# fwilliams/point-cloud-utils

Measured on AMD Instinct MI355X. Metric: query-points/s, Chamfer 1M-vs-1M fp32, higher is better.
Workload: dtype f32

## Files before the change

### point_cloud_utils_amd/csrc/grid2.h

```cpp
#pragma once
#include "grid.h"

namespace pcu {

constexpr int kPrepSamples = 1024;
constexpr int kXPartStride = 8;
constexpr int kStagedMaxBuckets = 2048;
constexpr int kFillWords = 2 * kStagedMaxBuckets + 8;

template <typename T>
struct CellMap {
    T org[3], inv_h; int G[3];
    __device__ __forceinline__ explicit CellMap(const GridParams<T>& g) {
#pragma unroll
        for (int j = 0; j < 3; ++j) { org[j] = uniform(g.org[j]); G[j] = uniform(g.G[j]); }
        inv_h = uniform(g.inv_h);
    }
    __device__ __forceinline__ unsigned cell(T x, T y, T z) const {
        const int cx = cell_coord(x, org[0], inv_h, G[0]), cy = cell_coord(y, org[1], inv_h, G[1]), cz = cell_coord(z, org[2], inv_h, G[2]);
        return (unsigned)row_run_lo(G[0], grid_row(G[1], cy, cz), cx, cx);
    }
};

__device__ __forceinline__ unsigned hash32(unsigned x) { x ^= x >> 16; x *= 0x7feb352du; x ^= x >> 15; x *= 0x846ca68bu; x ^= x >> 16; return x; }
// ... 285 lines not shown
        T rng6[6];
        const SampleOf<T> smp = sample_request<T>(a, a.n, tid);
        layout_from_sample<T>(a, a.n, smp, s_col, s_fin, &s_fresh, rng6);
        if (tid == 0) {
            GridGeo<T> f;
            for (int j = 0; j < 3; ++j) { f.org[j] = s_fresh.org[j]; f.slack[j] = s_fresh.slack[j]; f.G[j] = s_fresh.G[j]; f.rlo[j] = rng6[j]; f.rhi[j] = rng6[3 + j]; }
            f.h = s_fresh.h; f.inv_h = s_fresh.inv_h; f.ncells = s_fresh.ncells;
            if (a.geo_in) {
                const GridGeo<T> u = *a.geo_in;
                bool stale = false;
                for (int j = 0; j < 3; ++j) {
                    const T eu = u.rhi[j] - u.rlo[j], ef = f.rhi[j] - f.rlo[j], ext = eu > ef ? eu : ef, tol = (T)0.05 * ext;
                    const T dl = f.rlo[j] - u.rlo[j], dh = f.rhi[j] - u.rhi[j];
                    if (!((dl < (T)0 ? -dl : dl) <= tol) || !((dh < (T)0 ? -dh : dh) <= tol)) stale = true;
                }
                const T hr = f.h / u.h;
                if (!(hr > (T)0.96 && hr < (T)1.04)) stale = true;
                s_stale = stale ? 1 : 0;
            }
            *a.geo_out = f;
        }
        __syncthreads();
    }
    for (int i = tid; i < a.n_zero_next; i += kSortThreads) a.zero_next[i] = 0ull;
    for (int i = tid; i < a.n_zero2; i += kSortThreads) a.zero2[i] = 0u;
    T lo[3] = {Limits<T>::max_v, Limits<T>::max_v, Limits<T>::max_v};
    T hi[3] = {-Limits<T>::max_v, -Limits<T>::max_v, -Limits<T>::max_v};
    unsigned nf = 0;
    for (int b = tid; b < a.n_xpart; b += kSortThreads) {
#pragma unroll
        for (int j = 0; j < 3; ++j) {
            const T p = a.xpartial[(size_t)b * kXPartStride + j], q = a.xpartial[(size_t)b * kXPartStride + 3 + j];
            lo[j] = p < lo[j] ? p : lo[j]; hi[j] = q > hi[j] ? q : hi[j];
        }
        nf |= (unsigned)a.xpartial[(size_t)b * kXPartStride + 6];
    }
#pragma unroll
    for (int j = 0; j < 3; ++j) {
        const T p = wave_min63(lo[j]), q = wave_max63(hi[j]);
        if (lane == 63) { s_lo[wave][j] = p; s_hi[wave][j] = q; }
    }
    { const unsigned m = wave_or63(nf); if (lane == 63) s_nf[wave] = m; }
    __syncthreads();
    if (tid != 0) return;
    GridParams<T>* gp = a.gp;
    unsigned m = 0;
    for (int w = 0; w < kSortThreads / 64; ++w) m |= s_nf[w];
    const unsigned pinf = (m >> 1) & 7u, ninf = (m >> 4) & 7u;
    gp->nonfinite = ((m & 1u) ? kNfNaN : 0) | ((pinf & ninf) ? kNfBothInf : 0) | ((pinf | ninf) ? kNfAnyInf : 0) | (int)(m << 8);
    for (int j = 0; j < 3; ++j) {
        T p = s_lo[0][j], q = s_hi[0][j];
        for (int w = 1; w < kSortThreads / 64; ++w) { p = s_lo[w][j] < p ? s_lo[w][j] : p; q = s_hi[w][j] > q ? s_hi[w][j] : q; }
        if (!(p <= q)) { p = 0; q = 0; }
        gp->gmin[j] = p; gp->gmax[j] = q;
    }
    gp->has_large = (*a.ovf ? 2 : 0) | (s_stale ? kGeoStale : 0);
    if (a.n_large) *a.n_large = 0u;
    put_sentinels(a.sorted, a.n);
}

constexpr int kHeadTrips = (kStagedMaxBuckets + kSortThreads - 1) / kSortThreads;
template <typename T>
__device__ __forceinline__ void sort2_head_request(const Build2Side<T>& a, const int b, unsigned long long (&fw)[kHeadTrips]) {
#pragma unroll
    for (int q = 0; q < kHeadTrips; ++q) { const int i = q * kSortThreads + (int)threadIdx.x; fw[q] = i < b ? a.fill[i] : 0ull; }
}
__device__ __forceinline__ unsigned sort2_head_fold(const unsigned long long (&fw)[kHeadTrips], unsigned* const s_cnt, const int CB, unsigned* const s_w) {
    const int tid = threadIdx.x, lane = tid & 63, wave = tid >> 6;
    unsigned part = 0;
#pragma unroll
    for (int q = 0; q < kHeadTrips; ++q) part += (unsigned)(fw[q] >> 32);
#pragma unroll
    for (int o = 32; o > 0; o >>= 1) part += __shfl_xor(part, o, 64);
    if (lane == 0) s_w[wave] = part;
    for (int i = tid; i < CB; i += kSortThreads) s_cnt[i] = 0u;
    __syncthreads();
    unsigned s = 0;
    for (int w = 0; w < kSortThreads / 64; ++w) s += s_w[w];
    __syncthreads();
    return s;
}

constexpr int kRegIters = (kStageRecs + kSortThreads - 1) / kSortThreads;
template <typename T, bool FAST>
__device__ __forceinline__ void sort2_body(const int b, const Build2Side<T>& a, const int cnt_cap, const unsigned long long (&hw)[kHeadTrips], const unsigned pf, const unsigned nvalid,
                                           unsigned* const s_cnt, Pt4<T>* const s_stage, unsigned* const s_w, unsigned long long* const s_q, long long t_prev) {
    GridParams<T>* const gp = a.gp;
    const CellMap<T> cm(*gp);
    const int ncells = uniform(gp->ncells);
    const int shift = a.shift, CB = 1 << shift;
    const int NB = (ncells + CB - 1) >> shift;
    const int tid = threadIdx.x, lane = tid & 63, wave = tid >> 6;
    long long* const prof = a.prof;
#define S2_PROF(slot) do { if (prof && tid == 0) { const long long t_now = wall_clock64(); atomicAdd((unsigned long long*)&prof[slot], (unsigned long long)(t_now - t_prev)); t_prev = t_now; } } while (0)
    const unsigned cap = a.cap;
    const unsigned c0 = (unsigned)b << shift;
    const int ncl = min(CB, ncells - (int)c0);
    const Pt4<T>* const slot = a.tmp + (size_t)b * cap;
    const unsigned lastp = pf ? pf - 1u : 0u;
    typedef typename RawRec<T>::type Raw;
    constexpr int kIters = FAST ? kRegIters : kSortIters;
    constexpr int kSortBatch = 4;
    Raw recs[FAST ? kRegIters : 1];
    unsigned rr[kIters];
    if (FAST) {
        const Raw* const rslot = reinterpret_cast<const Raw*>(slot);
#pragma unroll
        for (int u = 0; u < kRegIters; ++u) recs[u] = rslot[min((unsigned)(u * kSortThreads + tid), lastp)];
    }
    const unsigned s = sort2_head_fold(hw, s_cnt, CB, s_w);
    const unsigned e = s + nvalid;
    S2_PROF(0);
    if (FAST) {
#pragma unroll
        for (int u = 0; u < kRegIters; ++u) {
            const unsigned p = (unsigned)(u * kSortThreads + tid);
            const Pt4<T>& rec = reinterpret_cast<const Pt4<T>&>(recs[u]);
            rr[u] = 0xffffffffu;
            if (p < pf && rec.idx >= 0) {
                const unsigned c = cm.cell(rec.x, rec.y, rec.z) - c0;
                rr[u] = (c << 16) | atomicAdd(&s_cnt[c], 1u);
            }
        }
    } else {
#pragma unroll
        for (int it0 = 0; it0 < kIters; it0 += kSortBatch) {
            Pt4<T> rec[kSortBatch];
            const bool batch_on = (unsigned)(it0 * kSortThreads) < pf;
            if (batch_on) {
#pragma unroll
                for (int u = 0; u < kSortBatch; ++u) rec[u] = slot[min((unsigned)((it0 + u) * kSortThreads + tid), lastp)];
            }
#pragma unroll
            for (int u = 0; u < kSortBatch; ++u) {
                const unsigned p = (unsigned)((it0 + u) * kSortThreads + tid);
                rr[it0 + u] = 0xffffffffu;
                if (batch_on && p < pf && rec[u].idx >= 0) {
                    const unsigned c = cm.cell(rec[u].x, rec[u].y, rec[u].z) - c0;
                    rr[it0 + u] = (c << 16) | atomicAdd(&s_cnt[c], 1u);
                }
            }
        }
    }
    __syncthreads();
    S2_PROF(1);
    const int per = CB >= kSortThreads ? CB / kSortThreads : 1;
    const int i0 = tid * per;
    {
        unsigned v[kBkMaxCellsPerBucket / kSortThreads], sum = 0; unsigned long long sq = 0;
#pragma unroll
        for (int q = 0; q < kBkMaxCellsPerBucket / kSortThreads; ++q) {
            v[q] = (q < per && i0 + q < CB) ? s_cnt[i0 + q] : 0u;
            sum += v[q]; sq += (unsigned long long)v[q] * v[q];
        }
        unsigned inc = sum;
#pragma unroll
        for (int o = 1; o < 64; o <<= 1) { const unsigned t = __shfl_up(inc, o, 64); if (lane >= o) inc += t; }
#pragma unroll
        for (int o = 32; o > 0; o >>= 1) sq += __shfl_xor(sq, o, 64);
        if (lane == 63) s_w[wave] = inc;
        if (lane == 0) s_q[wave] = sq;
        __syncthreads();
        if (tid == 0) {
            unsigned run = 0; unsigned long long Q = 0;
            for (int w = 0; w < kSortThreads / 64; ++w) { const unsigned t = s_w[w]; s_w[w] = run; run += t; Q += s_q[w]; }
            if (Q) atomicAdd(&gp->sumsq, Q);
            if (b == NB - 1) a.cell_start[ncells] = e;
        }
        __syncthreads();
        unsigned ex = inc - sum + s_w[wave];
#pragma unroll
        for (int q = 0; q < kBkMaxCellsPerBucket / kSortThreads; ++q) {
            if (q < per && i0 + q < CB) {
                s_cnt[i0 + q] = ex;
                if (i0 + q < ncl) a.cell_start[c0 + i0 + q] = s + ex;
                ex += v[q];
            }
        }
    }
    __syncthreads();
    S2_PROF(2);
    const int n_pts = a.n;
    T* const xyz = xyz_of(a.sorted, n_pts);
    int* const idx32 = idx32_of(a.sorted, n_pts);
    if (!FAST) {
#pragma unroll
        for (int it0 = 0; it0 < kIters; it0 += kSortBatch) {
            if (!((unsigned)(it0 * kSortThreads) < pf)) break;
            Pt4<T> rec[kSortBatch];
#pragma unroll
            for (int u = 0; u < kSortBatch; ++u) rec[u] = slot[min((unsigned)((it0 + u) * kSortThreads + tid), lastp)];
#pragma unroll
            for (int u = 0; u < kSortBatch; ++u) {
                const unsigned r = rr[it0 + u];
                if (r != 0xffffffffu) {
                    const unsigned pos = s + s_cnt[r >> 16] + (r & 0xffffu);
                    if (a.want_pt4) a.sorted[pos] = rec[u];
                    put_xyz(a.sorted, n_pts, pos, rec[u]);
                }
            }
        }
        return;
    }
    constexpr unsigned V = 16 / sizeof(T);
    T* const st = reinterpret_cast<T*>(s_stage);
    int* const sidx0 = reinterpret_cast<int*>(st + (V + 3 * kStageRecs + V - 1) / V * V);
    static_assert(((V + 3 * kStageRecs + V - 1) / V * V) * sizeof(T) + ((size_t)kStageRecs + 4) * 4 <= (size_t)kStageRecs * sizeof(Pt4<T>) + 64, "both streams fit the stage (bucket_sort_lds_bytes)");
    const unsigned phase = (unsigned)((3ull * (unsigned long long)s) & (V - 1));
    const unsigned iph = (unsigned)((reinterpret_cast<size_t>(idx32 + s) >> 2) & 3u);
    int* const sidx = sidx0 + iph;
    {
#pragma unroll
        for (int u = 0; u < kRegIters; ++u) {
            const unsigned r = rr[u];
            if (r != 0xffffffffu) {
                const Pt4<T>& rec = reinterpret_cast<const Pt4<T>&>(recs[u]);
                const unsigned pos = s_cnt[r >> 16] + (r & 0xffffu);
                T* const o = st + phase + 3u * pos;
                o[0] = rec.x; o[1] = rec.y; o[2] = rec.z; sidx[pos] = (int)rec.idx;
            }
        }
    }
    __syncthreads();
    S2_PROF(3);
    if (a.want_pt4) {
        for (unsigned i = tid; i < nvalid; i += kSortThreads) { Pt4<T> r; const T* const o = st + phase + 3u * i; r.x = o[0]; r.y = o[1]; r.z = o[2]; r.idx = sidx[i]; a.sorted[s + i] = r; }
    }
    {
        const unsigned end = phase + 3u * nvalid;
        T* const out = xyz + (3 * (size_t)s - phase);
        const unsigned v0 = (phase + V - 1) / V, v1 = end / V;
        for (unsigned c = v0 + tid; c < v1; c += kSortThreads)
            store16_wt(reinterpret_cast<Chunk16*>(out) + c, reinterpret_cast<const Chunk16*>(st)[c]);
        if (tid < V) {
            const unsigned La = phase + tid;
            if (La < min(v0 * V, end)) out[La] = st[La];
            const unsigned Lb = max(v1 * V, v0 * V) + tid;
            if (v1 >= v0 && Lb < end) out[Lb] = st[Lb];
        }
    }
    {
        const unsigned iend = iph + nvalid;
        int* const iout = idx32 + s - iph;
        const unsigned w0 = (iph + 3u) / 4u, w1 = iend / 4u;
        for (unsigned c = w0 + tid; c < w1; c += kSortThreads)
            store16_wt(reinterpret_cast<Chunk16*>(iout) + c, reinterpret_cast<const Chunk16*>(sidx0)[c]);
        if (tid >= 64 && tid < 68) {
            const unsigned t = (unsigned)tid - 64u;
            const unsigned La = iph + t;
            if (La < min(w0 * 4u, iend)) iout[La] = sidx0[La];
            const unsigned Lb = max(w1 * 4u, w0 * 4u) + t;
            if (w1 >= w0 && Lb < iend) iout[Lb] = sidx0[Lb];
        }
    }
    S2_PROF(4);
    if (prof) { asm volatile("s_waitcnt vmcnt(0)" ::: "memory"); S2_PROF(5); if (tid == 0) atomicAdd((unsigned long long*)&prof[7], 1ull); }
#undef S2_PROF
}

template <typename T>
__device__ __forceinline__ void sort2_bucket(const int b, const Build2Side<T>& a, const int cnt_cap) {
    extern __shared__ __attribute__((aligned(32))) unsigned char s_dyn[];
    unsigned* const s_cnt = reinterpret_cast<unsigned*>(s_dyn);
    Pt4<T>* const s_stage = reinterpret_cast<Pt4<T>*>(s_dyn + (size_t)cnt_cap * 4);
    __shared__ unsigned s_w[kSortThreads / 64 + 1];
    __shared__ unsigned long long s_q[kSortThreads / 64];
    if (*a.ovf) return;
    const int CB = 1 << a.shift;
    const int NB = (uniform(a.gp->ncells) + CB - 1) >> a.shift;
    if (b >= NB) return;
    long long t_prev = a.prof ? wall_clock64() : 0;
    const unsigned long long fw = a.fill[b];
    unsigned long long hw[kHeadTrips];
    sort2_head_request<T>(a, b, hw);
    const unsigned pf = min((unsigned)uniform(fw), a.cap), nvalid = (unsigned)(uniform(fw) >> 32);
    static_assert(kSortThreads * kSortIters >= kLargeBucket, "one trip per record of a full slot");
    if (pf <= (unsigned)(kRegIters * kSortThreads) && nvalid <= (unsigned)kStageRecs) sort2_body<T, true>(b, a, cnt_cap, hw, pf, nvalid, s_cnt, s_stage, s_w, s_q, t_prev);
    else sort2_body<T, false>(b, a, cnt_cap, hw, pf, nvalid, s_cnt, s_stage, s_w, s_q, t_prev);
}

template <typename T>
__global__ __launch_bounds__(kSortThreads) void k_bucket_sort2(const Build2Args<T> p, int nb0, int nb1, int cnt_cap, int nfold) {
    const int bid = (int)blockIdx.x;
    if (bid < nfold) { fold_xpartials<T>(p.a[bid]); return; }
    const int b = bid - nfold;
    const int side = b >= nb0 ? 1 : 0;
    sort2_bucket<T>(side ? b - nb0 : b, p.a[side], cnt_cap);
}

template <typename T>
struct Pt4Side { Pt4<T>* sorted; int n; };
template <typename T>
__global__ __launch_bounds__(kBlock) void k_make_pt4(const Pt4Side<T> a0, const Pt4Side<T> a1, int nb0) {
    const bool second = (int)blockIdx.x >= nb0;
    const Pt4Side<T>& a = second ? a1 : a0;
    const int nblk = second ? (int)gridDim.x - nb0 : nb0, bid = second ? (int)blockIdx.x - nb0 : (int)blockIdx.x;
    const T* const xyz = xyz_of(a.sorted, a.n);
    const int* const idx32 = idx32_of(a.sorted, a.n);
    for (int i = bid * kBlock + (int)threadIdx.x; i < a.n + 8; i += nblk * kBlock) {
        Pt4<T> r; r.x = xyz[3 * (size_t)i]; r.y = xyz[3 * (size_t)i + 1]; r.z = xyz[3 * (size_t)i + 2]; r.idx = idx32[i];
        a.sorted[i] = r;
    }
}

}
```

### point_cloud_utils_amd/csrc/index_host.h

```cpp
#pragma once

template <typename T>
struct GridIndex {
    GridParams<T>* gp = nullptr;
    unsigned* cell_start = nullptr;
    Pt4<T>* sorted = nullptr;
    unsigned* cell_of = nullptr; unsigned* rank = nullptr; unsigned* block_sums = nullptr;
    T* bbox_partial = nullptr;
    int n = 0, max_cells = 0, scan_blocks = 0;
    bool bucketed = false; int shift = 0, nb_max = 0, n_zero = 0;
    double h_want = 0.0;
    Pt4<T>* tmp = nullptr; unsigned *bucket_total = nullptr, *bucket_start = nullptr, *block_base = nullptr, *large_list = nullptr, *n_large = nullptr;
    bool one_pass = false;
    T* xpartial = nullptr;
    bool lean = false;
    const T* src = nullptr; double occ_built = 0.0;
    bool shared_grid = false;
};

static int max_cells_for(int64_t n, double occ) {
    double c = (double)n / (occ > 0 ? occ : 1.0) * 1.25 + 64.0;
    if (c > 64.0 * 1024 * 1024) c = 64.0 * 1024 * 1024;
    return (int)c;
}
// ... 25 lines not shown
    if (aalloc(a, &g.cell_start, (size_t)g.max_cells + 1 + kBkMaxBuckets + 8 + 64)) return -1;
    g.cell_start += 64;
    if (a.alloc((void**)&g.sorted, sorted_records_bytes((size_t)n, sizeof(Pt4<T>), sizeof(T)))) return -1;
    if (aalloc(a, &g.cell_of, (size_t)n)) return -1;
    if (aalloc(a, &g.rank, (size_t)n)) return -1;
    if (aalloc(a, &g.block_sums, (size_t)g.scan_blocks + 1)) return -1;
    if (aalloc(a, &g.bbox_partial, (size_t)kBboxBlocks * kBboxStride)) return -1;
    g.n_zero = g.max_cells + 1;
    if (g.bucketed) {
        g.bucket_total = g.cell_start + g.max_cells + 1; g.n_large = g.bucket_total + g.nb_max; g.n_zero = g.max_cells + 1 + g.nb_max + 1;
        g.one_pass = one_pass;
        if (aalloc(a, &g.tmp, one_pass ? std::max((size_t)n, (size_t)g.nb_max * kLargeBucket) : (size_t)n)) return -1;
        if (aalloc(a, &g.bucket_start, (size_t)g.nb_max + 1) || aalloc(a, &g.large_list, (size_t)g.nb_max + 1)) return -1;
        if (aalloc(a, &g.block_base, (size_t)((n + kBkBlockPts - 1) / kBkBlockPts) * g.nb_max)) return -1;
        if (one_pass && aalloc(a, &g.xpartial, (size_t)((n + 2047) / 2048) * kXPartStride)) return -1;
    }
    return 0;
}
template <typename T>
static size_t index_bytes(int64_t n, double occ) {
    ArenaState count; count.cap = ~(size_t)0 >> 1;
    Arena a(&count); GridIndex<T> g;
    (void)index_alloc(a, g, n, occ, IndexFor::OnePass);
    return count.off;
}
template <typename T>
static void index_same_form(GridIndex<T>& a, GridIndex<T>& b) {
    if (a.bucketed && b.bucketed && a.one_pass != b.one_pass) a.one_pass = b.one_pass = false;
}

template <typename T>
static GridSide<T> grid_side(const GridIndex<T>& g) {
    GridSide<T> r{};
    r.gp = g.gp; r.partial = g.bbox_partial; r.nparts = kBboxBlocks; r.n = g.n; r.occupancy = g.occ_built; r.max_cells = g.max_cells;
    r.sentinel = g.sorted + g.n; r.h_want = g.h_want; r.pts = g.src;
    return r;
}
template <typename T>
static BboxSide<T> bbox_side(const GridIndex<T>& g, void* zero2, int n_zero2) {
    BboxSide<T> r{};
    r.pts = g.src; r.n = g.n; r.partial = g.bbox_partial; r.counts = g.cell_start; r.n_counts = g.n_zero;
    r.zero2 = (unsigned*)zero2; r.n_zero2 = n_zero2; r.gp = g.gp;
    return r;
}
template <typename T>
static BucketSide<T> bucket_side(const GridIndex<T>& g) {
    BucketSide<T> r{};
    r.pts = g.src; r.n = g.n; r.gp = g.gp; r.shift = g.shift; r.nb_stride = g.nb_max;
    r.bucket_total = g.bucket_total; r.block_base = g.block_base; r.bucket_start = g.bucket_start; r.tmp = g.tmp; r.cell_start = g.cell_start; r.rank_tmp = g.rank;
    r.sorted = g.sorted; r.large_list = g.large_list; r.n_large = g.n_large; r.cap = g.one_pass ? kLargeBucket : 0u;
    return r;
}
template <typename T>
static LargeJob<T> large_job(const GridIndex<T>& g) {
    LargeJob<T> r{};
    r.gp = g.gp; r.bucket_start = g.bucket_start; r.large_list = g.large_list; r.n_large = g.n_large;
    r.tmp = g.tmp; r.rank_tmp = g.rank; r.cell_start = g.cell_start; r.sorted = g.sorted; r.n_pts = g.n;
    return r;
}
template <typename T>
static void build2_side(Build2Side<T>& r, const GridIndex<T>& g, int k, int bpts, unsigned long long* fw) {
    r = Build2Side<T>{};
    r.pts = g.src; r.n = g.n; r.gp = g.gp; r.shift = g.shift;
    r.occupancy = g.occ_built; r.max_cells = g.max_cells; r.h_want = g.h_want;
    r.fill = fw + (size_t)k * kStagedMaxBuckets; r.ovf = fw + 2 * kStagedMaxBuckets + k;
    r.tmp = g.tmp; r.cap = kLargeBucket;
    r.xpartial = g.xpartial; r.n_xpart = (g.n + bpts - 1) / bpts;
    r.cell_start = g.cell_start; r.sorted = g.sorted; r.want_pt4 = g.lean ? 0 : 1;
    r.n_large = g.n_large;
    r.spts0 = g.src; r.sn0 = g.n; r.spts1 = nullptr; r.sn1 = 0; r.n_layout = g.n;
}

struct StageTimer {
    const bool on; const int words;
    long long* dev = nullptr;
    StageTimer(const char* env, int nwords) : on(getenv(env) != nullptr), words(nwords) {}
    long long* arg() const { return on ? dev : nullptr; }
    int arm(hipStream_t s) {
        if (!on) return 0;
        if (!dev) HIP_TRY(hipMalloc((void**)&dev, words * sizeof(long long)));
        HIP_TRY(hipMemsetAsync(dev, 0, words * sizeof(long long), s));
        return 0;
    }
    int report(hipStream_t s, const char* tag, int count, std::initializer_list<const char*> stages) {
        if (!on) return 0;
        long long h[16]; HIP_TRY(hipMemcpyAsync(h, dev, words * sizeof(long long), hipMemcpyDeviceToHost, s)); HIP_WAIT(s);
        const double nb = h[count] > 0 ? (double)h[count] * 100.0 : 100.0;
        fprintf(stderr, "[%s prof] blocks %lld | mean us per block:", tag, h[count]);
        int i = 0;
        for (const char* st : stages) { fprintf(stderr, "%s%s %.2f", i ? "  " : " ", st, h[i] / nb); ++i; }
        fprintf(stderr, "\n");
        return 0;
    }
};

enum class BuildForm { Atomic, TwoPass, OnePass, Staged };
struct BuildChoice {
    BuildForm form[2];
    bool grid_in_scatter;
    int pts;
};
template <typename T>
static BuildChoice index_build_choose(const GridIndex<T>& a, const GridIndex<T>* b, const pcu_hip_ctx* ctx) {
    auto form_of = [](const GridIndex<T>& g) { return !g.bucketed ? BuildForm::Atomic : (g.one_pass ? BuildForm::OnePass : BuildForm::TwoPass); };
    BuildChoice ch{{form_of(a), form_of(b ? *b : a)}, false, 0};
    static const bool grid_kernel = getenv("PCU_HIP_GRID_KERNEL") != nullptr;
    ch.grid_in_scatter = !grid_kernel && ch.form[0] == BuildForm::OnePass && ch.form[1] == BuildForm::OnePass;
    static const bool build_v1 = getenv("PCU_HIP_BUILD_V1") != nullptr || getenv("PCU_HIP_PROF_BUILD") != nullptr;
    const int run_floor = 12 * std::max(a.nb_max, b ? b->nb_max : 0);
    if (!(ch.grid_in_scatter && !build_v1 && ctx && ctx->fill2 && a.xpartial && (!b || b->xpartial) && a.nb_max <= kStagedMaxBuckets &&
          (!b || b->nb_max <= kStagedMaxBuckets) && kBkThreads * StagedPts<T>::n >= run_floor)) return ch;
    ch.form[0] = ch.form[1] = BuildForm::Staged;
    ch.pts = StagedPts<T>::n;
    const long long ntot = (long long)a.n + (b ? b->n : 0);
    static const int n_cu = [] { hipDeviceProp_t pr; int d = 0; (void)hipGetDevice(&d); return hipGetDeviceProperties(&pr, d) == hipSuccess ? pr.multiProcessorCount : 256; }();
    while (ch.pts > 2 && (ntot + (long long)kBkThreads * ch.pts - 1) / ((long long)kBkThreads * ch.pts) < n_cu / 16 && kBkThreads * (ch.pts / 2) >= run_floor) ch.pts /= 2;
    return ch;
}

struct BuildOpts {
    bool defer_large = false;
    void* zero2 = nullptr; int n_zero2 = 0;
    pcu_hip_ctx* ctx = nullptr;
    bool keep_layout = false;
};

template <typename T>
static bool geo_match(pcu_hip_ctx* ctx, const GridIndex<T>& a, const GridIndex<T>& b, bool shared, Build2Side<T>& s0, Build2Side<T>& s1) {
    static const bool geo_off = getenv("PCU_HIP_NO_GEO_CACHE") != nullptr;
    if (geo_off || !ctx->geo.dev || a.n < kPrepSamples || b.n < kPrepSamples) return false;
    pcu_hip_ctx::GeoCache& gc = ctx->geo;
    const double occa = a.occ_built, occb = b.occ_built;
    const bool hit = gc.valid[0] && gc.valid[1] && gc.n[0] == a.n && gc.n[1] == b.n && gc.occ == occa && occa == occb && gc.h_want == a.h_want && a.h_want == b.h_want &&
                     gc.max_cells == a.max_cells && a.max_cells == b.max_cells && gc.shared == shared && gc.n_layout == s0.n_layout && gc.tsize == (int)sizeof(T);
    static_assert(sizeof(GridGeo<T>) <= 256, "two layouts fit the context's block");
    GridGeo<T>* const g0 = reinterpret_cast<GridGeo<T>*>(gc.dev), *const g1 = reinterpret_cast<GridGeo<T>*>(gc.dev + 256);
    s0.geo_out = g0; s1.geo_out = g1;
    if (hit) { s0.geo_in = g0; s1.geo_in = g1; }
    DEBUG_SKEW("[layout] handed down: %d (n %d %d, shared %d)\n", (int)hit, a.n, b.n, (int)shared);
    gc.valid[0] = gc.valid[1] = false;
    gc.n[0] = a.n; gc.n[1] = b.n; gc.occ = occa; gc.h_want = a.h_want; gc.max_cells = a.max_cells; gc.shared = shared; gc.n_layout = s0.n_layout; gc.tsize = (int)sizeof(T);
    return occa == occb && a.h_want == b.h_want && a.max_cells == b.max_cells;
}
static void geo_commit(pcu_hip_ctx* ctx) { ctx->geo.valid[0] = ctx->geo.valid[1] = true; }

template <typename T>
static int index_build_staged(GridIndex<T>& a, GridIndex<T>* b, hipStream_t s, const BuildOpts& o, int pts) {
    pcu_hip_ctx* const ctx = o.ctx;
    unsigned long long* const fw = ctx->fill2 + (size_t)ctx->fill_parity * kFillWords;
    const int bpts = kBkThreads * pts;
    const int nbcap = (std::max(a.nb_max, b ? b->nb_max : 0) + 63) / 64 * 64;
    Build2Args<T> sa;
    Build2Side<T>& s0 = sa.a[0], &s1 = sa.a[1];
    build2_side(s0, a, 0, bpts, fw);
    s0.zero_next = ctx->fill2 + (size_t)(ctx->fill_parity ^ 1) * kFillWords; s0.n_zero_next = kFillWords;
    s0.zero2 = (unsigned*)o.zero2; s0.n_zero2 = o.n_zero2;
    if (b) build2_side(s1, *b, 1, bpts, fw); else s1 = s0;
    const bool shared = b && a.shared_grid && b->shared_grid && a.occ_built == b->occ_built && a.max_cells == b->max_cells && a.shift == b->shift && a.nb_max == b->nb_max &&
                        a.h_want == b->h_want && a.n >= kPrepSamples && b->n >= kPrepSamples;
    if (b) a.shared_grid = b->shared_grid = shared; else a.shared_grid = false;
    if (shared) {
        s0.spts0 = s1.spts0 = a.src; s0.sn0 = s1.sn0 = a.n; s0.spts1 = s1.spts1 = b->src; s0.sn1 = s1.sn1 = b->n;
        s0.n_layout = s1.n_layout = std::max(a.n, b->n);
    }
    const bool geo_arm = o.keep_layout && b && geo_match(ctx, a, *b, shared, s0, s1);
    const int c0 = s0.n_xpart, c1 = b ? s1.n_xpart : 0;
    static StageTimer prof("PCU_HIP_PROF_BUILD2", 16);
    if (int rc = prof.arm(s)) return rc;
    s0.prof = s1.prof = prof.arg();
    static std::atomic<unsigned long long> attr_set2[2];
    if (attr_unset_here(attr_set2[sizeof(T) == 4 ? 0 : 1])) {
        if (StagedPts<T>::n >= 8) HIP_TRY(hipFuncSetAttribute(reinterpret_cast<const void*>(&k_bucket_onepass3<T, 8>), hipFuncAttributeMaxDynamicSharedMemorySize, (int)onepass3_lds_bytes<T>(8)));
        HIP_TRY(hipFuncSetAttribute(reinterpret_cast<const void*>(&k_bucket_onepass3<T, 4>), hipFuncAttributeMaxDynamicSharedMemorySize, (int)onepass3_lds_bytes<T>(4)));
        HIP_TRY(hipFuncSetAttribute(reinterpret_cast<const void*>(&k_bucket_onepass3<T, 2>), hipFuncAttributeMaxDynamicSharedMemorySize, (int)onepass3_lds_bytes<T>(2)));
        HIP_TRY(hipFuncSetAttribute(reinterpret_cast<const void*>(&k_bucket_sort2<T>), hipFuncAttributeMaxDynamicSharedMemorySize,
                                    (int)bucket_sort_lds_bytes<T>(kBkMaxCellsPerBucket)));
    }
    const size_t lds1 = onepass3_lds_bytes<T>(pts, nbcap);
    if (pts == 8) hipLaunchKernelGGL((k_bucket_onepass3<T, 8>), dim3(c0 + c1), dim3(kBkThreads), lds1, s, sa, c0, nbcap);
    else if (pts == 4) hipLaunchKernelGGL((k_bucket_onepass3<T, 4>), dim3(c0 + c1), dim3(kBkThreads), lds1, s, sa, c0, nbcap);
    else hipLaunchKernelGGL((k_bucket_onepass3<T, 2>), dim3(c0 + c1), dim3(kBkThreads), lds1, s, sa, c0, nbcap);
    if (int rc = prof.report(s, "onepass3", 15, {"layout", "points in", "keys+ranks", "scan+reservations", "staging", "run copies", "drain"})) return rc;
    const int t0 = a.nb_max, t1 = b ? b->nb_max : 0;
    const int cnt_cap = 1 << std::max(a.shift, b ? b->shift : 0);
    if (int rc = prof.arm(s)) return rc;
    hipLaunchKernelGGL(k_bucket_sort2<T>, dim3(t0 + t1 + (b ? 2 : 1)), dim3(kSortThreads), bucket_sort_lds_bytes<T>(cnt_cap), s, sa, t0, t1, cnt_cap, b ? 2 : 1);
    ctx->fill_parity ^= 1;
    if (int rc = prof.report(s, "sort2", 7, {"head", "load+rank", "scan", "place", "copies", "drain"})) return rc;
    HIP_TRY(hipGetLastError());
    if (geo_arm) geo_commit(ctx);
    return 0;
}

template <typename T>
static void index_large_pass(const GridIndex<T>& a, const GridIndex<T>* b, hipStream_t s) {
    const bool ua = a.bucketed, ub = b && b->bucketed;
    if (!ua && !ub) return;
    const LargeJob<T> ja = large_job(ua ? a : *b), jb = large_job(ua && ub ? *b : (ua ? a : *b));
    hipLaunchKernelGGL(k_bucket_large<T>, dim3(4 * kBboxBlocks), dim3(kBlock), 0, s, ja, jb, (ua && ub) ? 2 : 1);
    if (ua) (void)hipMemsetAsync(reinterpret_cast<char*>(a.gp) + offsetof(GridParams<T>, has_large), 0, sizeof(int), s);
    if (ub) (void)hipMemsetAsync(reinterpret_cast<char*>(b->gp) + offsetof(GridParams<T>, has_large), 0, sizeof(int), s);
}
template <typename T>
static int index_build_bucketed(const GridIndex<T>& a, const GridIndex<T>* b, hipStream_t s, const BuildOpts& o) {
    const GridIndex<T>* bs[2]; int nbs = 0;
    if (a.bucketed) bs[nbs++] = &a;
    if (b && b->bucketed) bs[nbs++] = b;
    if (!nbs) return 0;
    const BucketSide<T> s0 = bucket_side(*bs[0]), s1 = nbs > 1 ? bucket_side(*bs[1]) : s0;
    const int c0 = (bs[0]->n + kBkBlockPts - 1) / kBkBlockPts, c1 = nbs > 1 ? (bs[1]->n + kBkBlockPts - 1) / kBkBlockPts : 0;
    static StageTimer prof_onepass("PCU_HIP_PROF_BUILD", 8), prof_sort("PCU_HIP_PROF_BUILD", 8);
    if (int rc = prof_sort.arm(s)) return rc;
    const bool one_pass = bs[0]->one_pass;
    if (one_pass) {
        if (int rc = prof_onepass.arm(s)) return rc;
        hipLaunchKernelGGL(k_bucket_onepass<T>, dim3(c0 + c1), dim3(kBkThreads), 0, s, s0, s1, c0, prof_onepass.arg(), grid_side(*bs[0]), grid_side(*bs[nbs - 1]));
        if (int rc = prof_onepass.report(s, "onepass", 7, {"zero+loads", "keys+LDS ranks", "slot reservations", "stores"})) return rc;
    }
    else {
        hipLaunchKernelGGL(k_bucket_count<T>, dim3(c0 + c1), dim3(kBkThreads), 0, s, s0, s1, c0);
        hipLaunchKernelGGL(k_bucket_scatter<T>, dim3(c0 + c1), dim3(kBkThreads), 0, s, s0, s1, c0);
    }
    const int t0 = bs[0]->nb_max, t1 = nbs > 1 ? bs[1]->nb_max : 0;
    const int cnt_cap = 1 << std::max(bs[0]->shift, nbs > 1 ? bs[1]->shift : 0);
    const size_t lds = bucket_sort_lds_bytes<T>(cnt_cap);
    static std::atomic<unsigned long long> attr_set[2];
    if (attr_unset_here(attr_set[sizeof(T) == 4 ? 0 : 1]))
        HIP_TRY(hipFuncSetAttribute(reinterpret_cast<const void*>(&k_bucket_sort<T>), hipFuncAttributeMaxDynamicSharedMemorySize,
                                    (int)bucket_sort_lds_bytes<T>(kBkMaxCellsPerBucket)));
    hipLaunchKernelGGL(k_bucket_sort<T>, dim3(t0 + t1), dim3(kSortThreads), lds, s, s0, s1, t0, prof_sort.arg(), cnt_cap);
    if (int rc = prof_sort.report(s, "bucket_sort", 7, {"head", "zero+sync", "load+rank", "scan", "place"})) return rc;
    if (!o.defer_large && !one_pass) index_large_pass<T>(a, b, s);
    return 0;
}

template <typename T>
static void index_atomic_passes(const GridIndex<T>& g, const T* d_pts, hipStream_t s, bool closed = false) {
    const int n = g.n, nb = (n + kBlock - 1) / kBlock;
    hipLaunchKernelGGL(k_count<T>, dim3(nb), dim3(kBlock), 0, s, d_pts, n, g.gp, g.cell_of, g.rank, g.cell_start);
    hipLaunchKernelGGL(k_scan_reduce<T>, dim3(g.scan_blocks), dim3(kBlock), 0, s, g.cell_start, g.gp, g.block_sums);
    hipLaunchKernelGGL(k_scan_apply<T>, dim3(g.scan_blocks), dim3(kBlock), 0, s, g.cell_start, g.gp, g.block_sums, closed ? 0xffffffffu : (unsigned)n);
    hipLaunchKernelGGL(k_scatter<T>, dim3(nb), dim3(kBlock), 0, s, d_pts, n, g.cell_of, g.rank, g.cell_start, g.sorted);
}

template <typename T>
static int index_build_pair(GridIndex<T>& a, const T* pa, double occa, GridIndex<T>* b, const T* pb, double occb, hipStream_t s, const BuildOpts& o = BuildOpts()) {
    a.src = pa; a.occ_built = occa;
    if (b) { b->src = pb; b->occ_built = occb; index_same_form(a, *b); }
    const BuildChoice ch = index_build_choose(a, b, o.ctx);
    if (ch.form[0] == BuildForm::Staged) return index_build_staged(a, b, s, o, ch.pts);
    a.lean = false; if (b) b->lean = false;
    a.shared_grid = false; if (b) b->shared_grid = false;
    const BboxSide<T> x0 = bbox_side(a, o.zero2, o.n_zero2), x1 = b ? bbox_side(*b, nullptr, 0) : x0;
    hipLaunchKernelGGL(k_bbox_partial<T>, dim3(b ? 2 * kBboxBlocks : kBboxBlocks), dim3(kBlock), 0, s, x0, x1, kBboxBlocks);
    if (!ch.grid_in_scatter) hipLaunchKernelGGL(k_make_grid<T>, dim3(b ? 2 : 1), dim3(kBlock), 0, s, grid_side(a), grid_side(b ? *b : a));
    if (int rc = index_build_bucketed(a, b, s, o)) return rc;
    if (!a.bucketed) index_atomic_passes(a, pa, s);
    if (b && !b->bucketed) index_atomic_passes(*b, pb, s);
    HIP_TRY(hipGetLastError());
    return 0;
}
template <typename T>
static int index_build(GridIndex<T>& g, const T* d_pts, double occ, hipStream_t s, const BuildOpts& o = BuildOpts()) {
    return index_build_pair<T>(g, d_pts, occ, nullptr, nullptr, 0.0, s, o);
}

template <typename T>
static int core_range_enqueue(Arena& ar, const GridIndex<T>& base, const T* d_pts, hipStream_t s, QuantState<T>** out_qs) {
    QuantState<T>* qs = nullptr; unsigned *partial = nullptr, *hist = nullptr;
    if (aalloc(ar, &qs, 1) || aalloc(ar, &partial, (size_t)kHistBlocks * 3 * (kHistBins + 2)) || aalloc(ar, &hist, 3 * (kHistBins + 2))) return -1;
    hipLaunchKernelGGL(k_quant_init<T>, dim3(1), dim3(64), 0, s, base.gp, qs);
// ... 34 lines not shown
```

Before: 17.23 billion.

## Pair two buckets per block in sort2 to overlap loads with scan/copy

```diff
diff --git a/point_cloud_utils_amd/csrc/grid2.h b/point_cloud_utils_amd/csrc/grid2.h
--- a/point_cloud_utils_amd/csrc/grid2.h
+++ b/point_cloud_utils_amd/csrc/grid2.h
@@ -391,148 +391,102 @@
 }
 
 constexpr int kRegIters = (kStageRecs + kSortThreads - 1) / kSortThreads;
-template <typename T, bool FAST>
-__device__ __forceinline__ void sort2_body(const int b, const Build2Side<T>& a, const int cnt_cap, const unsigned long long (&hw)[kHeadTrips], const unsigned pf, const unsigned nvalid,
-                                           unsigned* const s_cnt, Pt4<T>* const s_stage, unsigned* const s_w, unsigned long long* const s_q, long long t_prev) {
-    GridParams<T>* const gp = a.gp;
-    const CellMap<T> cm(*gp);
-    const int ncells = uniform(gp->ncells);
-    const int shift = a.shift, CB = 1 << shift;
-    const int NB = (ncells + CB - 1) >> shift;
+__device__ __forceinline__ bool sort2_fast(const unsigned pf, const unsigned nvalid) { return pf <= (unsigned)(kRegIters * kSortThreads) && nvalid <= (unsigned)kStageRecs; }
+template <typename T>
+__device__ __forceinline__ void sort2_slot_request(const Pt4<T>* const slot, const unsigned lastp, typename RawRec<T>::type (&recs)[kRegIters]) {
+    const typename RawRec<T>::type* const rslot = reinterpret_cast<const typename RawRec<T>::type*>(slot);
+#pragma unroll
+    for (int u = 0; u < kRegIters; ++u) recs[u] = rslot[min((unsigned)(u * kSortThreads) + threadIdx.x, lastp)];
+}
+template <typename T>
+__device__ __forceinline__ void sort2_rank_regs(const CellMap<T>& cm, const unsigned c0, const unsigned pf, const typename RawRec<T>::type (&recs)[kRegIters],
+                                                unsigned (&rr)[kRegIters], unsigned* const s_cnt) {
+#pragma unroll
+    for (int u = 0; u < kRegIters; ++u) {
+        const unsigned p = (unsigned)(u * kSortThreads) + threadIdx.x;
+        const Pt4<T>& rec = reinterpret_cast<const Pt4<T>&>(recs[u]);
+        rr[u] = 0xffffffffu;
+        if (p < pf && rec.idx >= 0) {
+            const unsigned c = cm.cell(rec.x, rec.y, rec.z) - c0;
+            rr[u] = (c << 16) | atomicAdd(&s_cnt[c], 1u);
+        }
+    }
+}
+template <typename T>
+__device__ __forceinline__ void sort2_scan(const Build2Side<T>& a, const int b, const int NB, const int ncells, const unsigned c0, const int ncl, const int CB,
+                                           const unsigned s, const unsigned e, unsigned* const s_cnt, unsigned* const s_w, unsigned long long* const s_q) {
     const int tid = threadIdx.x, lane = tid & 63, wave = tid >> 6;
-    long long* const prof = a.prof;
-#define S2_PROF(slot) do { if (prof && tid == 0) { const long long t_now = wall_clock64(); atomicAdd((unsigned long long*)&prof[slot], (unsigned long long)(t_now - t_prev)); t_prev = t_now; } } while (0)
-    const unsigned cap = a.cap;
-    const unsigned c0 = (unsigned)b << shift;
-    const int ncl = min(CB, ncells - (int)c0);
-    const Pt4<T>* const slot = a.tmp + (size_t)b * cap;
-    const unsigned lastp = pf ? pf - 1u : 0u;
-    typedef typename RawRec<T>::type Raw;
-    constexpr int kIters = FAST ? kRegIters : kSortIters;
-    constexpr int kSortBatch = 4;
-    Raw recs[FAST ? kRegIters : 1];
-    unsigned rr[kIters];
-    if (FAST) {
-        const Raw* const rslot = reinterpret_cast<const Raw*>(slot);
-#pragma unroll
-        for (int u = 0; u < kRegIters; ++u) recs[u] = rslot[min((unsigned)(u * kSortThreads + tid), lastp)];
-    }
-    const unsigned s = sort2_head_fold(hw, s_cnt, CB, s_w);
-    const unsigned e = s + nvalid;
-    S2_PROF(0);
-    if (FAST) {
-#pragma unroll
-        for (int u = 0; u < kRegIters; ++u) {
-            const unsigned p = (unsigned)(u * kSortThreads + tid);
-            const Pt4<T>& rec = reinterpret_cast<const Pt4<T>&>(recs[u]);
-            rr[u] = 0xffffffffu;
-            if (p < pf && rec.idx >= 0) {
-                const unsigned c = cm.cell(rec.x, rec.y, rec.z) - c0;
-                rr[u] = (c << 16) | atomicAdd(&s_cnt[c], 1u);
-            }
-        }
-    } else {
-#pragma unroll
-        for (int it0 = 0; it0 < kIters; it0 += kSortBatch) {
-            Pt4<T> rec[kSortBatch];
-            const bool batch_on = (unsigned)(it0 * kSortThreads) < pf;
-            if (batch_on) {
-#pragma unroll
-                for (int u = 0; u < kSortBatch; ++u) rec[u] = slot[min((unsigned)((it0 + u) * kSortThreads + tid), lastp)];
-            }
-#pragma unroll
-            for (int u = 0; u < kSortBatch; ++u) {
-                const unsigned p = (unsigned)((it0 + u) * kSortThreads + tid);
-                rr[it0 + u] = 0xffffffffu;
-                if (batch_on && p < pf && rec[u].idx >= 0) {
-                    const unsigned c = cm.cell(rec[u].x, rec[u].y, rec[u].z) - c0;
-                    rr[it0 + u] = (c << 16) | atomicAdd(&s_cnt[c], 1u);
-                }
-            }
-        }
-    }
-    __syncthreads();
-    S2_PROF(1);
     const int per = CB >= kSortThreads ? CB / kSortThreads : 1;
     const int i0 = tid * per;
-    {
-        unsigned v[kBkMaxCellsPerBucket / kSortThreads], sum = 0; unsigned long long sq = 0;
-#pragma unroll
-        for (int q = 0; q < kBkMaxCellsPerBucket / kSortThreads; ++q) {
-            v[q] = (q < per && i0 + q < CB) ? s_cnt[i0 + q] : 0u;
-            sum += v[q]; sq += (unsigned long long)v[q] * v[q];
-        }
-        unsigned inc = sum;
-#pragma unroll
-        for (int o = 1; o < 64; o <<= 1) { const unsigned t = __shfl_up(inc, o, 64); if (lane >= o) inc += t; }
-#pragma unroll
-        for (int o = 32; o > 0; o >>= 1) sq += __shfl_xor(sq, o, 64);
-        if (lane == 63) s_w[wave] = inc;
-        if (lane == 0) s_q[wave] = sq;
-        __syncthreads();
-        if (tid == 0) {
-            unsigned run = 0; unsigned long long Q = 0;
-            for (int w = 0; w < kSortThreads / 64; ++w) { const unsigned t = s_w[w]; s_w[w] = run; run += t; Q += s_q[w]; }
-            if (Q) atomicAdd(&gp->sumsq, Q);
-            if (b == NB - 1) a.cell_start[ncells] = e;
-        }
-        __syncthreads();
-        unsigned ex = inc - sum + s_w[wave];
-#pragma unroll
-        for (int q = 0; q < kBkMaxCellsPerBucket / kSortThreads; ++q) {
-            if (q < per && i0 + q < CB) {
-                s_cnt[i0 + q] = ex;
-                if (i0 + q < ncl) a.cell_start[c0 + i0 + q] = s + ex;
-                ex += v[q];
-            }
-        }
-    }
-    __syncthreads();
-    S2_PROF(2);
+    unsigned v[kBkMaxCellsPerBucket / kSortThreads], sum = 0; unsigned long long sq = 0;
+#pragma unroll
+    for (int q = 0; q < kBkMaxCellsPerBucket / kSortThreads; ++q) {
+        v[q] = (q < per && i0 + q < CB) ? s_cnt[i0 + q] : 0u;
+        sum += v[q]; sq += (unsigned long long)v[q] * v[q];
+    }
+    unsigned inc = sum;
+#pragma unroll
+    for (int o = 1; o < 64; o <<= 1) { const unsigned t = __shfl_up(inc, o, 64); if (lane >= o) inc += t; }
+#pragma unroll
+    for (int o = 32; o > 0; o >>= 1) sq += __shfl_xor(sq, o, 64);
+    if (lane == 63) s_w[wave] = inc;
+    if (lane == 0) s_q[wave] = sq;
+    __syncthreads();
+    if (tid == 0) {
+        unsigned run = 0; unsigned long long Q = 0;
+        for (int w = 0; w < kSortThreads / 64; ++w) { const unsigned t = s_w[w]; s_w[w] = run; run += t; Q += s_q[w]; }
+        if (Q) atomicAdd(&a.gp->sumsq, Q);
+        if (b == NB - 1) a.cell_start[ncells] = e;
+    }
+    __syncthreads();
+    unsigned ex = inc - sum + s_w[wave];
+#pragma unroll
+    for (int q = 0; q < kBkMaxCellsPerBucket / kSortThreads; ++q) {
+        if (q < per && i0 + q < CB) {
+            s_cnt[i0 + q] = ex;
+            if (i0 + q < ncl) a.cell_start[c0 + i0 + q] = s + ex;
+            ex += v[q];
+        }
+    }
+}
+template <typename T>
+struct Sort2Stage {
+    static constexpr unsigned V = 16 / sizeof(T);
+    T* st; int* sidx0; unsigned phase, iph;
+    __device__ __forceinline__ Sort2Stage(Pt4<T>* const s_stage, const unsigned s, const Build2Side<T>& a) {
+        st = reinterpret_cast<T*>(s_stage);
+        sidx0 = reinterpret_cast<int*>(st + (V + 3 * kStageRecs + V - 1) / V * V);
+        static_assert(((V + 3 * kStageRecs + V - 1) / V * V) * sizeof(T) + ((size_t)kStageRecs + 4) * 4 <= (size_t)kStageRecs * sizeof(Pt4<T>) + 64, "both streams fit the stage (bucket_sort_lds_bytes)");
+        phase = (unsigned)((3ull * (unsigned long long)s) & (V - 1));
+        iph = (unsigned)((reinterpret_cast<size_t>(idx32_of(a.sorted, a.n) + s) >> 2) & 3u);
+    }
+};
+template <typename T>
+__device__ __forceinline__ void sort2_place(const Sort2Stage<T>& sg, const typename RawRec<T>::type (&recs)[kRegIters], const unsigned (&rr)[kRegIters], const unsigned* const s_cnt) {
+    int* const sidx = sg.sidx0 + sg.iph;
+#pragma unroll
+    for (int u = 0; u < kRegIters; ++u) {
+        const unsigned r = rr[u];
+        if (r != 0xffffffffu) {
+            const Pt4<T>& rec = reinterpret_cast<const Pt4<T>&>(recs[u]);
+            const unsigned pos = s_cnt[r >> 16] + (r & 0xffffu);
+            T* const o = sg.st + sg.phase + 3u * pos;
+            o[0] = rec.x; o[1] = rec.y; o[2] = rec.z; sidx[pos] = (int)rec.idx;
+        }
+    }
+}
+template <typename T>
+__device__ __forceinline__ void sort2_copy_out(const Build2Side<T>& a, const Sort2Stage<T>& sg, const unsigned s, const unsigned nvalid) {
+    constexpr unsigned V = Sort2Stage<T>::V;
+    const int tid = threadIdx.x;
+    T* const st = sg.st;
+    int* const sidx0 = sg.sidx0;
+    const unsigned phase = sg.phase, iph = sg.iph;
     const int n_pts = a.n;
     T* const xyz = xyz_of(a.sorted, n_pts);
     int* const idx32 = idx32_of(a.sorted, n_pts);
-    if (!FAST) {
-#pragma unroll
-        for (int it0 = 0; it0 < kIters; it0 += kSortBatch) {
-            if (!((unsigned)(it0 * kSortThreads) < pf)) break;
-            Pt4<T> rec[kSortBatch];
-#pragma unroll
-            for (int u = 0; u < kSortBatch; ++u) rec[u] = slot[min((unsigned)((it0 + u) * kSortThreads + tid), lastp)];
-#pragma unroll
-            for (int u = 0; u < kSortBatch; ++u) {
-                const unsigned r = rr[it0 + u];
-                if (r != 0xffffffffu) {
-                    const unsigned pos = s + s_cnt[r >> 16] + (r & 0xffffu);
-                    if (a.want_pt4) a.sorted[pos] = rec[u];
-                    put_xyz(a.sorted, n_pts, pos, rec[u]);
-                }
-            }
-        }
-        return;
-    }
-    constexpr unsigned V = 16 / sizeof(T);
-    T* const st = reinterpret_cast<T*>(s_stage);
-    int* const sidx0 = reinterpret_cast<int*>(st + (V + 3 * kStageRecs + V - 1) / V * V);
-    static_assert(((V + 3 * kStageRecs + V - 1) / V * V) * sizeof(T) + ((size_t)kStageRecs + 4) * 4 <= (size_t)kStageRecs * sizeof(Pt4<T>) + 64, "both streams fit the stage (bucket_sort_lds_bytes)");
-    const unsigned phase = (unsigned)((3ull * (unsigned long long)s) & (V - 1));
-    const unsigned iph = (unsigned)((reinterpret_cast<size_t>(idx32 + s) >> 2) & 3u);
-    int* const sidx = sidx0 + iph;
-    {
-#pragma unroll
-        for (int u = 0; u < kRegIters; ++u) {
-            const unsigned r = rr[u];
-            if (r != 0xffffffffu) {
-                const Pt4<T>& rec = reinterpret_cast<const Pt4<T>&>(recs[u]);
-                const unsigned pos = s_cnt[r >> 16] + (r & 0xffffu);
-                T* const o = st + phase + 3u * pos;
-                o[0] = rec.x; o[1] = rec.y; o[2] = rec.z; sidx[pos] = (int)rec.idx;
-            }
-        }
-    }
-    __syncthreads();
-    S2_PROF(3);
     if (a.want_pt4) {
+        const int* const sidx = sidx0 + iph;
         for (unsigned i = tid; i < nvalid; i += kSortThreads) { Pt4<T> r; const T* const o = st + phase + 3u * i; r.x = o[0]; r.y = o[1]; r.z = o[2]; r.idx = sidx[i]; a.sorted[s + i] = r; }
     }
     {
@@ -562,8 +516,86 @@
             if (w1 >= w0 && Lb < iend) iout[Lb] = sidx0[Lb];
         }
     }
-    S2_PROF(4);
-    if (prof) { asm volatile("s_waitcnt vmcnt(0)" ::: "memory"); S2_PROF(5); if (tid == 0) atomicAdd((unsigned long long*)&prof[7], 1ull); }
+}
+
+template <typename T, bool FAST>
+__device__ __forceinline__ void sort2_body(const int b, const Build2Side<T>& a, const int cnt_cap, const unsigned long long (&hw)[kHeadTrips], const unsigned pf, const unsigned nvalid,
+                                           unsigned* const s_cnt, Pt4<T>* const s_stage, unsigned* const s_w, unsigned long long* const s_q, long long t_prev) {
+    GridParams<T>* const gp = a.gp;
+    const CellMap<T> cm(*gp);
+    const int ncells = uniform(gp->ncells);
+    const int shift = a.shift, CB = 1 << shift;
+    const int NB = (ncells + CB - 1) >> shift;
+    const int tid = threadIdx.x;
+    long long* const prof = a.prof;
+#define S2_PROF(slot) do { if (prof && tid == 0) { const long long t_now = wall_clock64(); atomicAdd((unsigned long long*)&prof[slot], (unsigned long long)(t_now - t_prev)); t_prev = t_now; } } while (0)
+    const unsigned cap = a.cap;
+    const unsigned c0 = (unsigned)b << shift;
+    const int ncl = min(CB, ncells - (int)c0);
+    const Pt4<T>* const slot = a.tmp + (size_t)b * cap;
+    const unsigned lastp = pf ? pf - 1u : 0u;
+    constexpr int kIters = FAST ? kRegIters : kSortIters;
+    constexpr int kSortBatch = 4;
+    typename RawRec<T>::type recs[FAST ? kRegIters : 1];
+    unsigned rr[kIters];
+    if constexpr (FAST) sort2_slot_request<T>(slot, lastp, recs);
+    const unsigned s = sort2_head_fold(hw, s_cnt, CB, s_w);
+    const unsigned e = s + nvalid;
+    S2_PROF(0);
+    if constexpr (FAST) {
+        sort2_rank_regs<T>(cm, c0, pf, recs, rr, s_cnt);
+    } else {
+#pragma unroll
+        for (int it0 = 0; it0 < kIters; it0 += kSortBatch) {
+            Pt4<T> rec[kSortBatch];
+            const bool batch_on = (unsigned)(it0 * kSortThreads) < pf;
+            if (batch_on) {
+#pragma unroll
+                for (int u = 0; u < kSortBatch; ++u) rec[u] = slot[min((unsigned)((it0 + u) * kSortThreads + tid), lastp)];
+            }
+#pragma unroll
+            for (int u = 0; u < kSortBatch; ++u) {
+                const unsigned p = (unsigned)((it0 + u) * kSortThreads + tid);
+                rr[it0 + u] = 0xffffffffu;
+                if (batch_on && p < pf && rec[u].idx >= 0) {
+                    const unsigned c = cm.cell(rec[u].x, rec[u].y, rec[u].z) - c0;
+                    rr[it0 + u] = (c << 16) | atomicAdd(&s_cnt[c], 1u);
+                }
+            }
+        }
+    }
+    __syncthreads();
+    S2_PROF(1);
+    sort2_scan<T>(a, b, NB, ncells, c0, ncl, CB, s, e, s_cnt, s_w, s_q);
+    __syncthreads();
+    S2_PROF(2);
+    if constexpr (!FAST) {
+        const int n_pts = a.n;
+#pragma unroll
+        for (int it0 = 0; it0 < kIters; it0 += kSortBatch) {
+            if (!((unsigned)(it0 * kSortThreads) < pf)) break;
+            Pt4<T> rec[kSortBatch];
+#pragma unroll
+            for (int u = 0; u < kSortBatch; ++u) rec[u] = slot[min((unsigned)((it0 + u) * kSortThreads + tid), lastp)];
+#pragma unroll
+            for (int u = 0; u < kSortBatch; ++u) {
+                const unsigned r = rr[it0 + u];
+                if (r != 0xffffffffu) {
+                    const unsigned pos = s + s_cnt[r >> 16] + (r & 0xffffu);
+                    if (a.want_pt4) a.sorted[pos] = rec[u];
+                    put_xyz(a.sorted, n_pts, pos, rec[u]);
+                }
+            }
+        }
+    } else {
+        const Sort2Stage<T> sg(s_stage, s, a);
+        sort2_place<T>(sg, recs, rr, s_cnt);
+        __syncthreads();
+        S2_PROF(3);
+        sort2_copy_out<T>(a, sg, s, nvalid);
+        S2_PROF(4);
+        if (prof) { asm volatile("s_waitcnt vmcnt(0)" ::: "memory"); S2_PROF(5); if (tid == 0) atomicAdd((unsigned long long*)&prof[7], 1ull); }
+    }
 #undef S2_PROF
 }
 
@@ -584,8 +616,81 @@
     sort2_head_request<T>(a, b, hw);
     const unsigned pf = min((unsigned)uniform(fw), a.cap), nvalid = (unsigned)(uniform(fw) >> 32);
     static_assert(kSortThreads * kSortIters >= kLargeBucket, "one trip per record of a full slot");
-    if (pf <= (unsigned)(kRegIters * kSortThreads) && nvalid <= (unsigned)kStageRecs) sort2_body<T, true>(b, a, cnt_cap, hw, pf, nvalid, s_cnt, s_stage, s_w, s_q, t_prev);
+    if (sort2_fast(pf, nvalid)) sort2_body<T, true>(b, a, cnt_cap, hw, pf, nvalid, s_cnt, s_stage, s_w, s_q, t_prev);
     else sort2_body<T, false>(b, a, cnt_cap, hw, pf, nvalid, s_cnt, s_stage, s_w, s_q, t_prev);
+}
+
+template <typename T> struct Sort2Pairs { static constexpr bool on = sizeof(T) == 4; };
+template <typename T>
+struct Sort2Geo {
+    int ncells, CB, NB, ncl; unsigned c0;
+    __device__ __forceinline__ Sort2Geo(const Build2Side<T>& a, const int b) {
+        ncells = uniform(a.gp->ncells); CB = 1 << a.shift; NB = (ncells + CB - 1) >> a.shift;
+        c0 = (unsigned)b << a.shift; ncl = min(CB, ncells - (int)c0);
+    }
+};
+template <typename T>
+__device__ __forceinline__ void sort2_two(const Build2Args<T>& p, const int iA, const int iB, const int nb0, const int W, const int cnt_cap) {
+    extern __shared__ __attribute__((aligned(32))) unsigned char s_dyn[];
+    unsigned* const s_cntA = reinterpret_cast<unsigned*>(s_dyn), *const s_cntB = s_cntA + cnt_cap;
+    Pt4<T>* const s_stage = reinterpret_cast<Pt4<T>*>(s_dyn + (size_t)cnt_cap * 8);
+    __shared__ unsigned s_w[kSortThreads / 64 + 1];
+    __shared__ unsigned long long s_q[kSortThreads / 64];
+    const int tid = threadIdx.x;
+    const Build2Side<T>& A = p.a[iA >= nb0 ? 1 : 0], &B = p.a[iB >= nb0 ? 1 : 0];
+    const int bA = iA >= nb0 ? iA - nb0 : iA, bB = iB >= nb0 ? iB - nb0 : iB;
+    const Sort2Geo<T> gA(A, bA), gB(B, bB);
+    const bool liveA = bA < gA.NB && !*A.ovf, liveB = iB < W && bB < gB.NB && !*B.ovf;
+    if (liveA && liveB) {
+        long long* const prof = A.prof;
+        long long t_prev = prof ? wall_clock64() : 0;
+#define S2_PROF(slot) do { if (prof && tid == 0) { const long long t_now = wall_clock64(); atomicAdd((unsigned long long*)&prof[slot], (unsigned long long)(t_now - t_prev)); t_prev = t_now; } } while (0)
+        typedef typename RawRec<T>::type Raw;
+        const unsigned long long fwA = A.fill[bA], fwB = B.fill[bB];
+        unsigned long long hwA[kHeadTrips], hwB[kHeadTrips];
+        Raw recsA[kRegIters], recsB[kRegIters];
+        unsigned rrA[kRegIters], rrB[kRegIters];
+        sort2_head_request<T>(A, bA, hwA);
+        sort2_head_request<T>(B, bB, hwB);
+        const Pt4<T>* const slotA = A.tmp + (size_t)bA * A.cap, *const slotB = B.tmp + (size_t)bB * B.cap;
+        const unsigned pfA = min((unsigned)uniform(fwA), A.cap), nvA = (unsigned)(uniform(fwA) >> 32);
+        const unsigned pfB = min((unsigned)uniform(fwB), B.cap), nvB = (unsigned)(uniform(fwB) >> 32);
+        if (sort2_fast(pfA, nvA) && sort2_fast(pfB, nvB)) {
+            const CellMap<T> cmA(*A.gp), cmB(*B.gp);
+            sort2_slot_request<T>(slotA, pfA ? pfA - 1u : 0u, recsA);
+            const unsigned sA = sort2_head_fold(hwA, s_cntA, gA.CB, s_w);
+            S2_PROF(8);
+            sort2_rank_regs<T>(cmA, gA.c0, pfA, recsA, rrA, s_cntA);
+            sort2_slot_request<T>(slotB, pfB ? pfB - 1u : 0u, recsB);
+            __syncthreads();
+            S2_PROF(9);
+            sort2_scan<T>(A, bA, gA.NB, gA.ncells, gA.c0, gA.ncl, gA.CB, sA, sA + nvA, s_cntA, s_w, s_q);
+            __syncthreads();
+            const Sort2Stage<T> sgA(s_stage, sA, A);
+            sort2_place<T>(sgA, recsA, rrA, s_cntA);
+            S2_PROF(10);
+            const unsigned sB = sort2_head_fold(hwB, s_cntB, gB.CB, s_w);
+            sort2_rank_regs<T>(cmB, gB.c0, pfB, recsB, rrB, s_cntB);
+            S2_PROF(11);
+            sort2_copy_out<T>(A, sgA, sA, nvA);
+            S2_PROF(12);
+            __syncthreads();
+            sort2_scan<T>(B, bB, gB.NB, gB.ncells, gB.c0, gB.ncl, gB.CB, sB, sB + nvB, s_cntB, s_w, s_q);
+            __syncthreads();
+            const Sort2Stage<T> sgB(s_stage, sB, B);
+            sort2_place<T>(sgB, recsB, rrB, s_cntB);
+            __syncthreads();
+            S2_PROF(13);
+            sort2_copy_out<T>(B, sgB, sB, nvB);
+            S2_PROF(14);
+            if (prof) { asm volatile("s_waitcnt vmcnt(0)" ::: "memory"); S2_PROF(15); if (tid == 0) atomicAdd((unsigned long long*)&prof[16], 1ull); }
+            return;
+        }
+#undef S2_PROF
+    }
+    if (liveA) sort2_bucket<T>(bA, A, cnt_cap);
+    __syncthreads();
+    if (liveB) sort2_bucket<T>(bB, B, cnt_cap);
 }
 
 template <typename T>
@@ -595,6 +700,13 @@
     const int b = bid - nfold;
     const int side = b >= nb0 ? 1 : 0;
     sort2_bucket<T>(side ? b - nb0 : b, p.a[side], cnt_cap);
+}
+template <typename T>
+__global__ __launch_bounds__(kSortThreads) void k_bucket_sort2_pairs(const Build2Args<T> p, int nb0, int nb1, int cnt_cap, int nfold) {
+    const int bid = (int)blockIdx.x;
+    if (bid < nfold) { fold_xpartials<T>(p.a[bid]); return; }
+    const int W = nb0 + nb1;
+    sort2_two<T>(p, bid - nfold, bid - nfold + (W + 1) / 2, nb0, W, cnt_cap);
 }
 
 template <typename T>
diff --git a/point_cloud_utils_amd/csrc/index_host.h b/point_cloud_utils_amd/csrc/index_host.h
--- a/point_cloud_utils_amd/csrc/index_host.h
+++ b/point_cloud_utils_amd/csrc/index_host.h
@@ -131,18 +131,22 @@
         HIP_TRY(hipMemsetAsync(dev, 0, words * sizeof(long long), s));
         return 0;
     }
-    int report(hipStream_t s, const char* tag, int count, std::initializer_list<const char*> stages) {
+    int report(hipStream_t s, const char* tag, int count, std::initializer_list<const char*> stages, int first = 0) {
         if (!on) return 0;
-        long long h[16]; HIP_TRY(hipMemcpyAsync(h, dev, words * sizeof(long long), hipMemcpyDeviceToHost, s)); HIP_WAIT(s);
+        long long h[24]; HIP_TRY(hipMemcpyAsync(h, dev, words * sizeof(long long), hipMemcpyDeviceToHost, s)); HIP_WAIT(s);
         const double nb = h[count] > 0 ? (double)h[count] * 100.0 : 100.0;
         fprintf(stderr, "[%s prof] blocks %lld | mean us per block:", tag, h[count]);
-        int i = 0;
-        for (const char* st : stages) { fprintf(stderr, "%s%s %.2f", i ? "  " : " ", st, h[i] / nb); ++i; }
+        int i = first;
+        for (const char* st : stages) { fprintf(stderr, "%s%s %.2f", i > first ? "  " : " ", st, h[i] / nb); ++i; }
         fprintf(stderr, "\n");
         return 0;
     }
 };
 
+static int sort_n_cu() {
+    static const int n = [] { hipDeviceProp_t pr; int d = 0; (void)hipGetDevice(&d); return hipGetDeviceProperties(&pr, d) == hipSuccess ? pr.multiProcessorCount : 256; }();
+    return n;
+}
 enum class BuildForm { Atomic, TwoPass, OnePass, Staged };
 struct BuildChoice {
     BuildForm form[2];
@@ -162,7 +166,7 @@
     ch.form[0] = ch.form[1] = BuildForm::Staged;
     ch.pts = StagedPts<T>::n;
     const long long ntot = (long long)a.n + (b ? b->n : 0);
-    static const int n_cu = [] { hipDeviceProp_t pr; int d = 0; (void)hipGetDevice(&d); return hipGetDeviceProperties(&pr, d) == hipSuccess ? pr.multiProcessorCount : 256; }();
+    static const int n_cu = sort_n_cu();
     while (ch.pts > 2 && (ntot + (long long)kBkThreads * ch.pts - 1) / ((long long)kBkThreads * ch.pts) < n_cu / 16 && kBkThreads * (ch.pts / 2) >= run_floor) ch.pts /= 2;
     return ch;
 }
@@ -214,7 +218,7 @@
     }
     const bool geo_arm = o.keep_layout && b && geo_match(ctx, a, *b, shared, s0, s1);
     const int c0 = s0.n_xpart, c1 = b ? s1.n_xpart : 0;
-    static StageTimer prof("PCU_HIP_PROF_BUILD2", 16);
+    static StageTimer prof("PCU_HIP_PROF_BUILD2", 24);
     if (int rc = prof.arm(s)) return rc;
     s0.prof = s1.prof = prof.arg();
     static std::atomic<unsigned long long> attr_set2[2];
@@ -224,6 +228,9 @@
         HIP_TRY(hipFuncSetAttribute(reinterpret_cast<const void*>(&k_bucket_onepass3<T, 2>), hipFuncAttributeMaxDynamicSharedMemorySize, (int)onepass3_lds_bytes<T>(2)));
         HIP_TRY(hipFuncSetAttribute(reinterpret_cast<const void*>(&k_bucket_sort2<T>), hipFuncAttributeMaxDynamicSharedMemorySize,
                                     (int)bucket_sort_lds_bytes<T>(kBkMaxCellsPerBucket)));
+        if constexpr (Sort2Pairs<T>::on)
+            HIP_TRY(hipFuncSetAttribute(reinterpret_cast<const void*>(&k_bucket_sort2_pairs<T>), hipFuncAttributeMaxDynamicSharedMemorySize,
+                                        (int)(bucket_sort_lds_bytes<T>(kBkMaxCellsPerBucket) + (size_t)kBkMaxCellsPerBucket * 4)));
     }
     const size_t lds1 = onepass3_lds_bytes<T>(pts, nbcap);
     if (pts == 8) hipLaunchKernelGGL((k_bucket_onepass3<T, 8>), dim3(c0 + c1), dim3(kBkThreads), lds1, s, sa, c0, nbcap);
@@ -233,9 +240,17 @@
     const int t0 = a.nb_max, t1 = b ? b->nb_max : 0;
     const int cnt_cap = 1 << std::max(a.shift, b ? b->shift : 0);
     if (int rc = prof.arm(s)) return rc;
-    hipLaunchKernelGGL(k_bucket_sort2<T>, dim3(t0 + t1 + (b ? 2 : 1)), dim3(kSortThreads), bucket_sort_lds_bytes<T>(cnt_cap), s, sa, t0, t1, cnt_cap, b ? 2 : 1);
+    static const int pair_env = [] { const char* e = getenv("PCU_HIP_SORT_PAIR"); return e ? atoi(e) : -1; }();
+    const int nfold = b ? 2 : 1, W = t0 + t1;
+    const bool lean = a.lean && (!b || b->lean);
+    const bool pair = Sort2Pairs<T>::on && (pair_env >= 0 ? pair_env != 0 : lean && W + nfold > sort_n_cu());
+    if constexpr (Sort2Pairs<T>::on) {
+        if (pair) hipLaunchKernelGGL(k_bucket_sort2_pairs<T>, dim3(nfold + (W + 1) / 2), dim3(kSortThreads), bucket_sort_lds_bytes<T>(cnt_cap) + (size_t)cnt_cap * 4, s, sa, t0, t1, cnt_cap, nfold);
+    }
+    if (!pair) hipLaunchKernelGGL(k_bucket_sort2<T>, dim3(nfold + W), dim3(kSortThreads), bucket_sort_lds_bytes<T>(cnt_cap), s, sa, t0, t1, cnt_cap, nfold);
     ctx->fill_parity ^= 1;
     if (int rc = prof.report(s, "sort2", 7, {"head", "load+rank", "scan", "place", "copies", "drain"})) return rc;
+    if (pair) if (int rc = prof.report(s, "sort2 pairs", 16, {"A head", "A rank, B requested", "A scan+place", "B ranked", "A copies", "B scan+place", "B copies", "drain"}, 8)) return rc;
     HIP_TRY(hipGetLastError());
     if (geo_arm) geo_commit(ctx);
     return 0;
```

Result: faster. 17.51 billion, median of 6 (+1.6%).
